# NickTravers/NeuralNetworkLibrary

Hardware: AMD Instinct MI355X
Metric: ResNet-34 224x224 training throughput (Learner.train1minibatch, fwd+loss+bwd+optimizer) (higher is better)
Workload: dtype f32; 1 GPU; DogsCats ResNet-34 classifier, 224x224, bs=64 per GPU, SGD momentum 0.9, fp32; global_batch=64, image_size=224, parallelism=dp1

## Files before the change

### include/nnl.h

```cpp
#ifndef NNL_H_
#define NNL_H_

#include <stddef.h>
#include <stdint.h>

#ifdef __cplusplus
extern "C" {
#endif

typedef enum {
  NNL_OK = 0,
  NNL_ERR_INVALID_ARG = -1,
  NNL_ERR_HIP = -2,
  NNL_ERR_UNSUPPORTED = -3,
  NNL_ERR_WORKSPACE = -4
} nnl_status_t;

int nnl_version(void);
const char* nnl_last_error(void);
int nnl_reload_env(void);

enum { NNL_PROF_CONV_FWD = 0, NNL_PROF_CONV_DGRAD = 1, NNL_PROF_CONV_WGRAD = 2, NNL_PROF_EMBDOT = 3,
       NNL_PROF_TABULAR = 4, NNL_PROF_RETINA_LOSS = 5, NNL_PROF_LSTM = 6, NNL_PROF_SOFTMAX_CE = 7,
       NNL_PROF_ELEMENTWISE = 8, NNL_PROF_GEMM = 9, NNL_PROF_OPTIM = 10, NNL_PROF_KINDS = 11 };
// ... 48 lines not shown
int nnl_conv2d_wino_preferred(const nnl_conv_geom_t* g, int dgrad);
int nnl_wino_filter_multi(const nnl_wino_desc_t* desc, const int32_t* block_desc, int64_t n_blocks, void* stream);
int nnl_conv2d_fwd_pre(const float* x, const float* w, const float* bias, float* y, const nnl_conv_geom_t* g, int relu,
                       void* workspace, size_t workspace_bytes, int32_t* tile_counters, float* bn_partials, const float* bn_pivot,
                       int32_t* bn_rows, const float* u, void* stream);
int nnl_conv2d_dgrad_pre(const float* dy, const float* wt, float* dx, const nnl_conv_geom_t* g, const float* addend,
                         void* workspace, size_t workspace_bytes, int32_t* tile_counters, const float* u, void* stream);
size_t nnl_debug_conv_wino_workspace_bytes(int N, int H, int W, int C, int K);
int nnl_debug_conv_wino_fwd(const float* x, const float* filt, const float* bias, const float* add, float* y, void* ws,
                            size_t ws_bytes, int32_t* counters, long n_counters, float* bn_part, const float* bn_pivot, int N,
                            int H, int W, int C, int K, int relu, int flip, void* stream);
size_t nnl_debug_conv_wino2_workspace_bytes(int N, int H, int W, int C, int K);
int nnl_debug_conv_wino2_fwd(const float* x, const float* filt, const float* bias, const float* add, float* y, void* ws,
                            size_t ws_bytes, int32_t* counters, long n_counters, float* bn_part, const float* bn_pivot, int N,
                            int H, int W, int C, int K, int relu, int flip, void* stream);
int nnl_debug_conv_plan_times(int N, int H, int W, int C, int K, double* out);
size_t nnl_conv2d_wgrad_workspace_bytes(const nnl_conv_geom_t* g);
int nnl_conv2d_wgrad(const float* x, const float* dy, float* dw, const nnl_conv_geom_t* g, void* workspace,
                     size_t workspace_bytes, void* stream);
size_t nnl_colsum_workspace_bytes(int64_t rows, int64_t cols);
int nnl_sum_tensors(const float* const* src, int n, float* out, int64_t numel, void* stream);
int nnl_colsum(const float* a, float* out, int64_t rows, int64_t cols, void* workspace, size_t workspace_bytes,
               void* stream);
int nnl_relu_gate_colsum(const float* dy, const float* y, float* g, float* colsum, int64_t rows, int64_t cols, void* workspace,
                         size_t workspace_bytes, void* stream);
int nnl_act_gate_colsum(const float* dy, const float* y, float* g, float* colsum, int64_t rows, int64_t cols, int act,
                        void* workspace, size_t workspace_bytes, void* stream);

size_t nnl_bn_workspace_bytes(int64_t rows, int64_t C);
int nnl_bn_fwd(const float* x, const float* gamma, const float* beta, const float* residual, float* y,
// ... 141 lines not shown
```

### neuralnetworklibrary_amd/_lib.py

```python
import ctypes as C
import os

import torch

_HERE = os.path.dirname(os.path.abspath(__file__))
LIB_PATH = os.environ.get('NNL_LIB_PATH') or os.path.join(_HERE, 'libnnl_hip.so')

if not os.path.exists(LIB_PATH):
    raise ImportError(
        f"{LIB_PATH} not found: build it with `python -c 'import __graft_entry__ as g; g.build()'` "
        "(or `make -C neuralnetworklibrary_amd/csrc`). There is no CPU fallback for the HIP hot path.")

lib = C.CDLL(LIB_PATH)

c_p = C.c_void_p
i32, i64, f32, f64 = C.c_int32, C.c_int64, C.c_float, C.c_double
sz = C.c_size_t


class ConvGeom(C.Structure):
    _fields_ = [('N', i32), ('H', i32), ('W', i32), ('C', i32), ('K', i32), ('R', i32), ('S', i32),
                ('stride', i32), ('pad', i32), ('P', i32), ('Q', i32)]


# ... 12 lines not shown
                                     c_p, c_p]),
    'nnl_embdotbias_bwd_workspace_bytes': (sz, [i64]),
    'nnl_embdotbias_bwd': (C.c_int, [c_p, c_p, c_p, c_p, c_p, c_p, c_p, c_p, c_p, i64, i64, i64, i64, C.c_int,
                                     f32, f32, c_p, sz, c_p]),
    'nnl_conv2d_fwd_workspace_bytes': (sz, [C.POINTER(ConvGeom)]),
    'nnl_conv2d_dgrad_workspace_bytes': (sz, [C.POINTER(ConvGeom)]),
    'nnl_conv2d_tile_counters': (i64, []),
    'nnl_conv2d_wino_preferred': (C.c_int, [C.POINTER(ConvGeom), C.c_int]),
    'nnl_wino_filter_multi': (C.c_int, [c_p, c_p, i64, c_p]),
    'nnl_conv2d_fwd_pre': (C.c_int, [c_p, c_p, c_p, c_p, C.POINTER(ConvGeom), C.c_int, c_p, sz, c_p, c_p, c_p, C.POINTER(i32), c_p, c_p]),
    'nnl_conv2d_dgrad_pre': (C.c_int, [c_p, c_p, c_p, C.POINTER(ConvGeom), c_p, c_p, sz, c_p, c_p, c_p]),
    'nnl_debug_conv_wino_workspace_bytes': (sz, [C.c_int] * 5),
    'nnl_debug_conv_wino_fwd': (C.c_int, [c_p] * 6 + [sz, c_p, C.c_long, c_p, c_p] + [C.c_int] * 7 + [c_p]),
    'nnl_debug_conv_wino2_workspace_bytes': (sz, [C.c_int] * 5),
    'nnl_debug_conv_wino2_fwd': (C.c_int, [c_p] * 6 + [sz, c_p, C.c_long, c_p, c_p] + [C.c_int] * 7 + [c_p]),
    'nnl_debug_conv_plan_times': (C.c_int, [C.c_int] * 5 + [C.POINTER(C.c_double)]),
    'nnl_conv2d_fwd': (C.c_int, [c_p, c_p, c_p, c_p, C.POINTER(ConvGeom), C.c_int, c_p, sz, c_p, c_p, c_p, C.POINTER(i32), c_p]),
    'nnl_conv2d_weight_transpose': (C.c_int, [c_p, c_p, C.c_int, C.c_int, C.c_int, C.c_int, c_p]),
    'nnl_conv2d_weight_transpose_multi': (C.c_int, [c_p, c_p, i64, f64, c_p]),
    'nnl_conv2d_dgrad': (C.c_int, [c_p, c_p, c_p, C.POINTER(ConvGeom), c_p, c_p, sz, c_p, c_p]),
    'nnl_conv2d_wgrad_workspace_bytes': (sz, [C.POINTER(ConvGeom)]),
    'nnl_conv2d_wgrad': (C.c_int, [c_p, c_p, c_p, C.POINTER(ConvGeom), c_p, sz, c_p]),
    'nnl_colsum_workspace_bytes': (sz, [i64, i64]),
    'nnl_colsum': (C.c_int, [c_p, c_p, i64, i64, c_p, sz, c_p]),
    'nnl_relu_gate_colsum': (C.c_int, [c_p, c_p, c_p, c_p, i64, i64, c_p, sz, c_p]),
    'nnl_conv2d_fwd_add_up2': (C.c_int, [c_p, c_p, c_p, c_p, c_p, C.POINTER(ConvGeom), c_p]),
    'nnl_upsample2_bwd': (C.c_int, [c_p, c_p, i64, i64, i64, i64, c_p]),
    'nnl_act_gate_colsum': (C.c_int, [c_p, c_p, c_p, c_p, i64, i64, C.c_int, c_p, sz, c_p]),
    'nnl_maxpool2d_fwd': (C.c_int, [c_p, c_p, c_p, i64, i64, i64, i64, i64, i64, C.c_int, C.c_int, C.c_int, c_p]),
    'nnl_maxpool2d_bwd': (C.c_int, [c_p, c_p, c_p, i64, i64, i64, i64, i64, i64, C.c_int, C.c_int, C.c_int, c_p]),
# ... 121 lines not shown
```

### neuralnetworklibrary_amd/csrc/wino2.hip

```cpp
#include "wino.h"
#include "wino_filter.h"
#include "igemm_taps.h"
#include <algorithm>

namespace {

constexpr int kCUs = 256;

template <int POL>
__device__ __forceinline__ f32x4 buf_load4_spol(__amdgpu_buffer_rsrc_t rsrc, unsigned voff, unsigned soff) {
  const i32x4 v = __builtin_bit_cast(i32x4, __builtin_amdgcn_raw_buffer_load_b128(rsrc, (int)voff, (int)soff, POL));
  return __builtin_bit_cast(f32x4, v);
}

struct Wino2Params {
  const float* a;
  const float* b;
  float* y;
  const float* bias;
  const float* add;
  unsigned a_bytes, b_bytes;
  int H, W, C, H2, W2;
  int ch;
  int prio;
// ... 5 lines not shown
  int bal, main_ks, n_main_tiles, tail_slices, tail_row0;
  float* main_out; long main_slab_stride;
  float* tail_out; long tail_slab_stride;
  int* tile_counters;
  float* bn_part; const float* bn_pivot;
  int pos_cs;
};

__global__ void wino2_filter_kernel(const float* __restrict__ w, float* __restrict__ u, long KC, int C, int flip) {
  const long i = (long)blockIdx.x * blockDim.x + threadIdx.x;
  if (i >= KC) return;
  const long c = i % C, k = i / C;
  wino2_filter_item(w + k * 9 * C + c, u + k * 16 * C + c, C, flip);
}

template <int BK, int OCC, bool POS = false>
__global__ __launch_bounds__(256, OCC) void wino2_kernel(const Wino2Params p) {
  constexpr int BM = 64, BN = 64, BKP = BK + 4, KC = BK / 4, RPP = 256 / KC, PA = BM / RPP, PB = BN / RPP;
  __shared__ __attribute__((aligned(16))) float lds[2][(BM + BN) * BKP];
  const int tid = threadIdx.x, lane = tid & 63, wave = tid >> 6, wm = wave >> 1, wn = wave & 1;
  int logical, kslice = 0, nslices = 1, row0 = 0;
  bool in_tail = false;
  if (p.bal) {
    const int nmb = p.n_main_tiles * p.main_ks;
    if ((int)blockIdx.x < nmb) {
      const int u = nnl_xcd_remap(blockIdx.x, nmb);
      logical = u / p.main_ks;
      kslice = u - logical * p.main_ks;
      nslices = p.main_ks;
    } else {
      const int tb = (int)blockIdx.x - nmb;
      const int t = tb / p.tail_slices;
      kslice = tb - t * p.tail_slices;
      logical = p.n_main_tiles + t;
      nslices = p.tail_slices;
// ... 13 lines not shown
  int a_off[PA];
  unsigned rmask[PA], cmask[PA];
#pragma unroll
  for (int i = 0; i < PA; ++i) {
    const int m = m0 + lrow + i * RPP;
    const bool valid = m < p.M4;
    const int mm = valid ? m : 0;
    const int l2 = qdiv(mm, p.mg_W2), j = mm - l2 * p.W2;
    const int n = qdiv(l2, p.mg_H2), ii = l2 - n * p.H2;
    a_off[i] = (((n * p.H + 2 * ii - 1) * p.W + 2 * j - 1) * p.C + kc * 4) * 4;
    unsigned rm = 0, cm = 0;
    if (valid) {
      for (int a = 0; a < 4; ++a) if ((unsigned)(2 * ii - 1 + a) < (unsigned)p.H) rm |= 1u << a;
      for (int a = 0; a < 4; ++a) if ((unsigned)(2 * j - 1 + a) < (unsigned)p.W) cm |= 1u << a;
    }
    rmask[i] = rm; cmask[i] = cm;
  }
  unsigned b_off[PB];
#pragma unroll
  for (int i = 0; i < PB; ++i) {
    const int nr = n0 + lrow + i * RPP;
    b_off[i] = nr < p.Nc ? (unsigned)(nr * 16 * p.C + kc * 4) * 4u : 0xFFFFFFFFu;
  }
  unsigned v00[PA], v01[PA], v10[PA], v11[PA], b_tap = 0;
  float sr = 1.f, sc = 1.f;
  auto set_pos = [&](int t) {
    const int xi = t >> 2, nu = t & 3;
    const int ra_ = xi, rb_ = xi < 2 ? 2 : 1;
    const int ca = nu, cb = nu < 2 ? 2 : 1;
    sr = xi == 1 ? 1.f : -1.f;
    sc = nu == 1 ? 1.f : -1.f;
    b_tap = (unsigned)(t * p.C) * 4u;
    const int wc = p.W * p.C * 4, c4 = p.C * 4;
#pragma unroll
    for (int i = 0; i < PA; ++i) {
      const bool ra_ok = (rmask[i] >> ra_) & 1u, rb_ok = (rmask[i] >> rb_) & 1u;
      const bool ca_ok = (cmask[i] >> ca) & 1u, cb_ok = (cmask[i] >> cb) & 1u;
      v00[i] = (ra_ok && ca_ok) ? (unsigned)(a_off[i] + ra_ * wc + ca * c4) : 0xFFFFFFFFu;
      v01[i] = (ra_ok && cb_ok) ? (unsigned)(a_off[i] + ra_ * wc + cb * c4) : 0xFFFFFFFFu;
      v10[i] = (rb_ok && ca_ok) ? (unsigned)(a_off[i] + rb_ * wc + ca * c4) : 0xFFFFFFFFu;
      v11[i] = (rb_ok && cb_ok) ? (unsigned)(a_off[i] + rb_ * wc + cb * c4) : 0xFFFFFFFFu;
    }
  };
  f32x4 r00[PA], r01[PA], r10[PA], r11[PA], rb[PB];
  auto load_tile = [&](int c0) {
#pragma unroll
    for (int i = 0; i < PA; ++i) {
      r00[i] = buf_load4(ra_src, v00[i], (unsigned)c0 * 4u); r01[i] = buf_load4(ra_src, v01[i], (unsigned)c0 * 4u);
      r10[i] = buf_load4(ra_src, v10[i], (unsigned)c0 * 4u); r11[i] = buf_load4(ra_src, v11[i], (unsigned)c0 * 4u);
    }
#pragma unroll
    for (int i = 0; i < PB; ++i) rb[i] = buf_load4(rb_src, b_off[i], b_tap + (unsigned)c0 * 4u);
  };
  float sr_ld = 1.f, sc_ld = 1.f;
  auto store_tile = [&](int buf) {
    float* As = lds[buf];
    float* Bs = As + BM * BKP;
#pragma unroll
    for (int i = 0; i < PA; ++i) {
      f32x4 v;
#pragma unroll
      for (int e = 0; e < 4; ++e)
        v[e] = __builtin_fmaf(sr_ld, __builtin_fmaf(sc_ld, r11[i][e], r10[i][e]), __builtin_fmaf(sc_ld, r01[i][e], r00[i][e]));
      *reinterpret_cast<f32x4*>(As + (lrow + i * RPP) * BKP + kc * 4) = v;
    }
#pragma unroll
    for (int i = 0; i < PB; ++i) *reinterpret_cast<f32x4*>(Bs + (lrow + i * RPP) * BKP + kc * 4) = rb[i];
// ... 99 lines not shown
#pragma unroll
        for (int e = 0; e < 16; ++e) y10[e] = __builtin_fmaf(k10, tm[e], y10[e]);
      }
      if (k11 != 0.f) {
#pragma unroll
        for (int e = 0; e < 16; ++e) y11[e] = __builtin_fmaf(k11, tm[e], y11[e]);
      }
#pragma unroll
      for (int e = 0; e < 16; ++e) tm[e] = 0.f;
      cs_cur = 0; t_cur = (t_cur + 1) & 15;
    }
  }

  const int col_l = lane & 31, row_h = (lane >> 5) * 4;
  constexpr int kSc1 = 1 << 4;
  if constexpr (POS) {
    __shared__ int ticket;
    const long sstride = p.main_slab_stride;
    const __amdgpu_buffer_rsrc_t rs = __builtin_amdgcn_make_buffer_rsrc(p.main_out, 0, (int)((long)nslices * sstride * 4), 0x00020000);
    const int cl = n0 + wn * 32 + col_l;
#pragma unroll
    for (int e = 0; e < 16; ++e) {
      const int row = m0 + wm * 32 + (e & 3) + 8 * (e >> 2) + row_h;
      const long off = (long)kslice * sstride + (long)row * p.Nc + cl;
      const bool ok = row < p.M4 && cl < p.Nc;
      __builtin_amdgcn_raw_buffer_store_b32(__float_as_uint(tm[e]), rs, ok ? (int)(off * 4) : -1, 0, kSc1);
    }
    asm volatile("s_waitcnt vmcnt(0)" ::: "memory");
    __syncthreads();
    if (tid == 0) ticket = __hip_atomic_fetch_add(&p.tile_counters[logical], 1, __ATOMIC_RELAXED, __HIP_MEMORY_SCOPE_AGENT);
    __syncthreads();
    if (ticket != nslices - 1) return;
    if (tid == 0) __hip_atomic_store(&p.tile_counters[logical], 0, __ATOMIC_RELAXED, __HIP_MEMORY_SCOPE_AGENT);
    float fs1[4] = {0.f, 0.f, 0.f, 0.f}, fs2[4] = {0.f, 0.f, 0.f, 0.f};
    const int c4 = n0 + (tid & 15) * 4, cs = p.pos_cs;
    const int wrow = p.W * p.Nc;
    auto item_off = [&](int k4, bool& ok) {
      const int row = m0 + (tid >> 4) + 16 * k4;
      ok = row < p.M4 && c4 < p.Nc;
      return ok ? (unsigned)(((long)row * p.Nc + c4) * 4) : 0xFFFFFFFFu;
    };
    auto finish_item = [&](int k4, f32x4 (&m)[16]) {
      const int row = m0 + (tid >> 4) + 16 * k4;
      f32x4 r0[4], r1[4];
#pragma unroll
      for (int xi = 0; xi < 4; ++xi) {
        r0[xi] = (m[xi * 4 + 0] + m[xi * 4 + 1]) + m[xi * 4 + 2];
        r1[xi] = (m[xi * 4 + 1] - m[xi * 4 + 2]) + m[xi * 4 + 3];
      }
      f32x4 out[4];
      out[0] = (r0[0] + r0[1]) + r0[2];
      out[1] = (r1[0] + r1[1]) + r1[2];
      out[2] = (r0[1] - r0[2]) + r0[3];
      out[3] = (r1[1] - r1[2]) + r1[3];
      const int l2 = qdiv(row, p.mg_W2), j = row - l2 * p.W2;
      const int n = qdiv(l2, p.mg_H2), ii = l2 - n * p.H2;
      const long ob = (((long)n * p.H + 2 * ii) * p.W + 2 * j) * p.Nc + c4;
      const bool h1 = 2 * ii + 1 < p.H, w1 = 2 * j + 1 < p.W;
// ... 21 lines not shown
      f32x4 ma[16];
#pragma unroll
      for (int t = 0; t < 16; ++t) ma[t] = buf_load4_spol<kSc1>(rs, oa, (unsigned)((long)(t * cs) * sstride * 4));
      for (int sl = 1; sl < cs; ++sl) {
#pragma unroll
        for (int t0 = 0; t0 < 16; t0 += 8) {
          f32x4 pa[8];
#pragma unroll
          for (int t = 0; t < 8; ++t) pa[t] = buf_load4_spol<kSc1>(rs, oa, (unsigned)((long)((t0 + t) * cs + sl) * sstride * 4));
#pragma unroll
          for (int t = 0; t < 8; ++t) ma[t0 + t] += pa[t];
        }
      }
      finish_item(k4, ma);
    }
    if (p.bn_part) {
      __syncthreads();
      float* red = &lds[0][0];
#pragma unroll
      for (int e = 0; e < 4; ++e) {
        red[(((tid >> 4) * 64) + (tid & 15) * 4 + e) * 2 + 0] = fs1[e];
        red[(((tid >> 4) * 64) + (tid & 15) * 4 + e) * 2 + 1] = fs2[e];
      }
      __syncthreads();
      if (tid < 64 && n0 + tid < p.Nc) {
        float a = 0.f, b = 0.f;
        for (int r = 0; r < 16; ++r) { a += red[(r * 64 + tid) * 2]; b += red[(r * 64 + tid) * 2 + 1]; }
        p.bn_part[((long)tile_m * p.Nc + n0 + tid) * 2 + 0] = a;
        p.bn_part[((long)tile_m * p.Nc + n0 + tid) * 2 + 1] = b;
      }
    }
    return;
  }
  if (partial) {
    __shared__ int ticket;
    float* const base = in_tail ? p.tail_out : p.main_out;
    const long sstride = in_tail ? p.tail_slab_stride : p.main_slab_stride;
    const __amdgpu_buffer_rsrc_t rs = __builtin_amdgcn_make_buffer_rsrc(base, 0, (int)((long)nslices * sstride * 4), 0x00020000);
    const int cl = n0 + wn * 32 + col_l;
#pragma unroll
    for (int e = 0; e < 16; ++e) {
      const int row = m0 + wm * 32 + (e & 3) + 8 * (e >> 2) + row_h;
      const long off = (long)kslice * sstride + (long)(row - row0) * 4 * p.Nc + cl;
      const bool ok = row < p.M4 && cl < p.Nc;
      __builtin_amdgcn_raw_buffer_store_b32(__float_as_uint(y00[e]), rs, ok ? (int)(off * 4) : -1, 0, kSc1);
      __builtin_amdgcn_raw_buffer_store_b32(__float_as_uint(y01[e]), rs, ok ? (int)((off + p.Nc) * 4) : -1, 0, kSc1);
      __builtin_amdgcn_raw_buffer_store_b32(__float_as_uint(y10[e]), rs, ok ? (int)((off + 2 * p.Nc) * 4) : -1, 0, kSc1);
      __builtin_amdgcn_raw_buffer_store_b32(__float_as_uint(y11[e]), rs, ok ? (int)((off + 3 * p.Nc) * 4) : -1, 0, kSc1);
    }
    asm volatile("s_waitcnt vmcnt(0)" ::: "memory");
    __syncthreads();
    if (tid == 0) ticket = __hip_atomic_fetch_add(&p.tile_counters[logical], 1, __ATOMIC_RELAXED, __HIP_MEMORY_SCOPE_AGENT);
    __syncthreads();
    if (ticket != nslices - 1) return;
    if (tid == 0) __hip_atomic_store(&p.tile_counters[logical], 0, __ATOMIC_RELAXED, __HIP_MEMORY_SCOPE_AGENT);
    float fs1[4] = {0.f, 0.f, 0.f, 0.f}, fs2[4] = {0.f, 0.f, 0.f, 0.f};
    const int h = (tid >> 4) & 3, c4 = n0 + (tid & 15) * 4;
    for (int k16 = 0; k16 < 16; ++k16) {
      const int row = m0 + (tid >> 6) + 4 * k16;
      if (row >= p.M4 || c4 >= p.Nc) continue;
      const int l2 = qdiv(row, p.mg_W2), j = row - l2 * p.W2;
      const int n = qdiv(l2, p.mg_H2), ii = l2 - n * p.H2;
      const int oh = 2 * ii + (h >> 1), ow = 2 * j + (h & 1);
      if (oh >= p.H || ow >= p.W) continue;
      f32x4 v = {0.f, 0.f, 0.f, 0.f};
      for (int sl0 = 0; sl0 < nslices; sl0 += 8) {
        f32x4 part[8];
#pragma unroll
        for (int sl = 0; sl < 8; ++sl)
          if (sl0 + sl < nslices) part[sl] = buf_load4_pol(rs, (unsigned)(((long)(sl0 + sl) * sstride + ((long)(row - row0) * 4 + h) * p.Nc + c4) * 4), kSc1);
#pragma unroll
        for (int sl = 0; sl < 8; ++sl)
          if (sl0 + sl < nslices) v += part[sl];
      }
      const long o = (((long)n * p.H + oh) * p.W + ow) * p.Nc + c4;
      if (p.bias) v += *reinterpret_cast<const f32x4*>(p.bias + c4);
      if (p.add) v += *reinterpret_cast<const f32x4*>(p.add + o);
      if (p.relu == 1) { v[0] = fmaxf(v[0], 0.f); v[1] = fmaxf(v[1], 0.f); v[2] = fmaxf(v[2], 0.f); v[3] = fmaxf(v[3], 0.f); }
      *reinterpret_cast<f32x4*>(p.y + o) = v;
      if (p.bn_part) {
        const f32x4 pv = *reinterpret_cast<const f32x4*>(p.bn_pivot + c4);
#pragma unroll
        for (int e = 0; e < 4; ++e) { const float d = v[e] - pv[e]; fs1[e] += d; fs2[e] += d * d; }
      }
    }
    if (p.bn_part) {
      __syncthreads();
      float* red = &lds[0][0];
#pragma unroll
      for (int e = 0; e < 4; ++e) {
        red[(((tid >> 4) * 64) + (tid & 15) * 4 + e) * 2 + 0] = fs1[e];
        red[(((tid >> 4) * 64) + (tid & 15) * 4 + e) * 2 + 1] = fs2[e];
      }
      __syncthreads();
      if (tid < 64 && n0 + tid < p.Nc) {
        float a = 0.f, b = 0.f;
        for (int r = 0; r < 16; ++r) { a += red[(r * 64 + tid) * 2]; b += red[(r * 64 + tid) * 2 + 1]; }
        p.bn_part[((long)tile_m * p.Nc + n0 + tid) * 2 + 0] = a;
        p.bn_part[((long)tile_m * p.Nc + n0 + tid) * 2 + 1] = b;
      }
    }
    return;
  }
  constexpr int LDT = 68;
  float* tl = &lds[0][0];
  float fs1[4] = {0.f, 0.f, 0.f, 0.f}, fs2[4] = {0.f, 0.f, 0.f, 0.f};
  const int c4 = n0 + (tid & 15) * 4;
  int pb[4];
  unsigned okm[4];
#pragma unroll
  for (int k4 = 0; k4 < 4; ++k4) {
    const int row = m0 + (tid >> 4) + 16 * k4;
    const int l2 = qdiv(row, p.mg_W2), j = row - l2 * p.W2;
    const int n = qdiv(l2, p.mg_H2), ii = l2 - n * p.H2;
    pb[k4] = ((n * p.H + 2 * ii) * p.W + 2 * j) * p.Nc + c4;
    const bool ok = row < p.M4 && c4 < p.Nc, h1 = 2 * ii + 1 < p.H, w1 = 2 * j + 1 < p.W;
    okm[k4] = ok ? (1u | (w1 ? 2u : 0u) | (h1 ? 4u : 0u) | ((h1 && w1) ? 8u : 0u)) : 0u;
  }
  const int wrow = p.W * p.Nc;
#pragma unroll
  for (int h = 0; h < 4; ++h) {
    if (h) __syncthreads();
#pragma unroll
    for (int e = 0; e < 16; ++e)
      tl[(wm * 32 + (e & 3) + 8 * (e >> 2) + row_h) * LDT + wn * 32 + col_l] = h == 0 ? y00[e] : (h == 1 ? y01[e] : (h == 2 ? y10[e] : y11[e]));
    __syncthreads();
#pragma unroll
    for (int k4 = 0; k4 < 4; ++k4) {
      if (!((okm[k4] >> h) & 1u)) continue;
      f32x4 v = *reinterpret_cast<const f32x4*>(tl + ((tid >> 4) + 16 * k4) * LDT + (tid & 15) * 4);
      const int o = pb[k4] + (h >> 1) * wrow + (h & 1) * p.Nc;
      if (p.bias) v += *reinterpret_cast<const f32x4*>(p.bias + c4);
      if (p.add) v += *reinterpret_cast<const f32x4*>(p.add + o);
      if (p.relu == 1) { v[0] = fmaxf(v[0], 0.f); v[1] = fmaxf(v[1], 0.f); v[2] = fmaxf(v[2], 0.f); v[3] = fmaxf(v[3], 0.f); }
      *reinterpret_cast<f32x4*>(p.y + o) = v;
      if (p.bn_part) {
        const f32x4 pv = *reinterpret_cast<const f32x4*>(p.bn_pivot + c4);
#pragma unroll
        for (int e = 0; e < 4; ++e) { const float d = v[e] - pv[e]; fs1[e] += d; fs2[e] += d * d; }
      }
    }
  }
  if (p.bn_part) {
    __syncthreads();
    float* red = &lds[0][0];
#pragma unroll
    for (int e = 0; e < 4; ++e) {
      red[(((tid >> 4) * 64) + (tid & 15) * 4 + e) * 2 + 0] = fs1[e];
      red[(((tid >> 4) * 64) + (tid & 15) * 4 + e) * 2 + 1] = fs2[e];
    }
    __syncthreads();
    if (tid < 64 && n0 + tid < p.Nc) {
      float a = 0.f, b = 0.f;
      for (int r = 0; r < 16; ++r) { a += red[(r * 64 + tid) * 2]; b += red[(r * 64 + tid) * 2 + 1]; }
      p.bn_part[((long)tile_m * p.Nc + n0 + tid) * 2 + 0] = a;
      p.bn_part[((long)tile_m * p.Nc + n0 + tid) * 2 + 1] = b;
    }
  }
}

struct W2Plan {
  int bk, on, main_ks, n_main_tiles, tail_slices, tail_row0;
  size_t main_floats, tail_floats;
  double t_us;
  int pos_cs;
};

double w2_pos_cost(long T, long M4, int Nc, int C, int cs) {
  const double a = 0.363, b = 0.490, tfix = 4.0;
  const long occ = 4, nwg = T * 16 * cs, I = (C / 32) / cs;
  const long nb = nnl_cdiv(nwg, (long)kCUs);
  const double c = (double)(nb < occ ? nb : occ);
  const double slab_b = 2.0 * 16 * cs * (double)M4 * Nc * 4;
  return nb * I * (b + a / c) + tfix * nb / c + slab_b / 11.7e6 + (3.0 + 1.5 * cs) + 4.0;
}

double w2_cost(long T, long gn, long M4, int Nc, long I, int bk, int ks, int S, W2Plan* out) {
  const double a = bk == 32 ? 0.363 : 0.226, b = bk == 32 ? 0.490 : 0.243, tfix = bk == 32 ? 12.3 : 15.0;
  const long occ = bk == 16 ? 4 : 3;
  long n_main = ((T * ks / kCUs) * kCUs / ks / gn) * gn;
  if (n_main > T) n_main = T;
  const long tail = T - n_main;
  if (tail == 0 && S > 1) return -1.0;
  const long m = nnl_cdiv(n_main * ks, (long)kCUs), q = nnl_cdiv(tail * S, (long)kCUs);
  const long W = m * nnl_cdiv(I, (long)ks) + q * nnl_cdiv(I, (long)S), nb = m + q;
  const double c = (double)(nb < occ ? nb : occ);
  const long row0 = (n_main / gn) * 64 < M4 ? (n_main / gn) * 64 : M4;
  const double main_b = ks > 1 ? (2.0 * ks + 1) * row0 * 4 * Nc * 4 : 0;
  const double tail_b = (S > 1 && tail) ? (2.0 * S + 1) * (M4 - row0) * 4 * Nc * 4 : 0;
  if (out) {
    out->bk = bk; out->on = (ks > 1 || (S > 1 && tail)) ? 1 : 0;
    out->main_ks = ks; out->n_main_tiles = (int)n_main; out->tail_slices = tail ? S : 1; out->tail_row0 = (int)row0;
    out->main_floats = ks > 1 ? (size_t)ks * row0 * 4 * Nc : 0;
    out->tail_floats = (S > 1 && tail) ? (size_t)S * (M4 - row0) * 4 * Nc : 0;
  }
  return W * (b + a / c) + tfix * nb / c + (main_b + tail_b) / 11.7e6 + 10.0;
}

W2Plan wino2_plan(long M4, int Nc, int C) {
  W2Plan best{};
  const long gm = nnl_cdiv(M4, 64), gn = nnl_cdiv(Nc, 64), T = gm * gn;
  const int f_ks = NNL_ENV_INT("NNL_WINO_PLAN_KS", 0), f_S = NNL_ENV_INT("NNL_WINO_PLAN_S", 0);
  const bool balance = NNL_ENV_INT("NNL_WINO_BALANCE", 1) != 0;
  double best_t = 1e300;
  static const int kSlices[] = {1, 2, 3, 4, 6, 8, 12, 16};
  for (int bk = 16; bk <= 32; bk *= 2) {
    if (C % bk != 0) continue;
    const long I = 16L * (C / bk);
    for (int ks = 1; ks <= 4; ks *= 2) {
      if (ks > 1 && (!balance || I / ks < 8)) break;
      if (f_ks > 0 && ks != f_ks && balance) continue;
      for (int S : kSlices) {
        if (S > 1 && (!balance || I / S < 4)) break;
        W2Plan cand{};
        const double t = w2_cost(T, gn, M4, Nc, I, bk, ks, S, &cand);
        if (t < 0) break;
        if (f_S > 0 && balance && cand.n_main_tiles < T && S != f_S) continue;
        if (t < best_t) { best_t = t; best = cand; best.t_us = t; }
      }
    }
  }
  if (best_t == 1e300) {
    best.t_us = w2_cost(T, gn, M4, Nc, 16L * (C / 16), 16, 1, 1, &best);
    best_t = best.t_us;
  }
  const int e_pos = NNL_ENV_INT("NNL_WINO2_POS", -1);
  if (e_pos != 0 && (balance || e_pos > 0) && C % 32 == 0) {
    const int csteps = C / 32;
    double pt = 1e300; int pcs = 0;
    for (int cs = 1; cs <= 8; cs *= 2) {
      if (csteps % cs != 0 || (csteps / cs < 2 && cs > 1)) break;
      if (e_pos > 0 && cs != e_pos && csteps % e_pos == 0) continue;
      const size_t fl = (size_t)16 * cs * M4 * Nc;
      if (fl * sizeof(float) >= (1UL << 31)) break;
      const double t = w2_pos_cost(T, M4, Nc, C, cs);
      if (t < pt) { pt = t; pcs = cs; }
    }
    if (pcs && (e_pos > 0 || pt < best_t)) {
      best = W2Plan{};
      best.bk = 32; best.on = 1; best.main_ks = 16 * pcs; best.n_main_tiles = (int)T; best.tail_slices = 1; best.tail_row0 = (int)M4;
      best.main_floats = (size_t)16 * pcs * M4 * Nc; best.tail_floats = 0; best.t_us = pt; best.pos_cs = pcs;
    }
  }
  return best;
}

size_t align4(size_t floats) { return (floats + 3) & ~(size_t)3; }

long quads(int N, int H, int W) { return (long)N * ((H + 1) / 2) * ((W + 1) / 2); }

}

bool nnl_wino2_ok(int N, int H, int W, int Cin, int Nc, int R, int S, int stride, int pad) {
  if (R != 3 || S != 3 || stride != 1 || pad != 1 || W < 2 || H < 2 || Cin % 16 != 0 || Nc % 4 != 0) return false;
  const long a_b = (long)N * H * W * Cin * 4, b_b = (long)Nc * 16 * Cin * 4, y_b = (long)N * H * W * Nc * 4;
  if ((quads(N, H, W) + 128) * (long)std::max((W + 1) / 2, (H + 1) / 2) >= (1L << 32)) return false;
  return a_b < (1L << 31) && b_b < (1L << 31) && y_b < (1L << 31);
}

double nnl_wino2_plan_time_us(int N, int H, int W, int Cin, int Nc) { return wino2_plan(quads(N, H, W), Nc, Cin).t_us; }
bool nnl_wino2_plan_is_pos(int N, int H, int W, int Cin, int Nc) { return wino2_plan(quads(N, H, W), Nc, Cin).pos_cs > 0; }

size_t nnl_wino2_workspace_bytes(int N, int H, int W, int Cin, int Nc) {
  const W2Plan pl = wino2_plan(quads(N, H, W), Nc, Cin);
  return (align4((size_t)Nc * 16 * Cin) + (pl.on ? pl.main_floats + pl.tail_floats : 0)) * sizeof(float);
}

int nnl_wino2_bn_rows(int N, int H, int W) { return (int)nnl_cdiv(quads(N, H, W), 64L); }

int nnl_wino2_launch(const WinoProblem& q, void* ws, size_t ws_bytes, int* tile_counters, long n_counters, hipStream_t s) {
  const long M4 = quads(q.N, q.H, q.W);
  const size_t u_floats = align4((size_t)q.Nc * 16 * q.Cin);
  if (ws == nullptr || ws_bytes < u_floats * sizeof(float)) return nnl_set_error(NNL_ERR_WORKSPACE, "wino2: workspace too small");
  float* u = (float*)ws;
  if (q.u_pre == nullptr) {
    const long KC = (long)q.Nc * q.Cin;
// ... 1 lines not shown
    NNL_CHECK_LAUNCH();
  }
  Wino2Params p{};
  p.a = q.in; p.b = q.u_pre ? q.u_pre : u; p.y = q.out; p.bias = q.bias; p.add = q.add;
  p.a_bytes = (unsigned)((long)q.N * q.H * q.W * q.Cin * 4); p.b_bytes = (unsigned)((long)q.Nc * 16 * q.Cin * 4);
  {
    const int e_ch = NNL_ENV_INT("NNL_WINO2_CHUNK", 0);
    p.ch = (e_ch > 0 && e_ch % 32 == 0 && q.Cin % e_ch == 0) ? e_ch : q.Cin;
    p.prio = 0;
  }
  p.H = q.H; p.W = q.W; p.C = q.Cin; p.H2 = (q.H + 1) / 2; p.W2 = (q.W + 1) / 2; p.M4 = (int)M4; p.Nc = q.Nc; p.relu = q.relu;
  {
    auto magic = [](int d) { return d <= 1 ? 0u : (unsigned)(((1ULL << 32) + d - 1) / (unsigned)d); };
    p.mg_W2 = magic(p.W2); p.mg_H2 = magic(p.H2);
  }
  p.grid_m = (int)nnl_cdiv(M4, 64L); p.grid_n = (int)nnl_cdiv(q.Nc, 64);
  p.bn_part = q.bn_part; p.bn_pivot = q.bn_pivot;
  const long T = (long)p.grid_m * p.grid_n;
  W2Plan pl = wino2_plan(M4, q.Nc, q.Cin);
  if (pl.on && (tile_counters == nullptr || T > n_counters || ws_bytes < (u_floats + pl.main_floats + pl.tail_floats) * sizeof(float) ||
                pl.main_floats * sizeof(float) >= (1UL << 31) || pl.tail_floats * sizeof(float) >= (1UL << 31))) {
    if (pl.pos_cs) {
      const int bk = q.Cin % 32 == 0 ? 32 : 16;
      w2_cost(T, p.grid_n, M4, q.Nc, 16L * (q.Cin / bk), bk, 1, 1, &pl);
      pl.pos_cs = 0;
    }
    pl.on = 0;
  }
  unsigned grid = (unsigned)T;
  if (pl.pos_cs) {
    p.bal = 1; p.main_ks = pl.main_ks; p.n_main_tiles = pl.n_main_tiles; p.tail_slices = 1; p.tail_row0 = (int)M4;
    p.main_out = u + u_floats; p.main_slab_stride = M4 * q.Nc; p.tile_counters = tile_counters; p.pos_cs = pl.pos_cs;
    grid = (unsigned)(T * pl.main_ks);
    hipLaunchKernelGGL((wino2_kernel<32, 4, true>), dim3(grid), dim3(256), 0, s, p);
    NNL_CHECK_LAUNCH();
    return NNL_OK;
  }
  if (pl.on) {
    p.bal = 1; p.main_ks = pl.main_ks; p.n_main_tiles = pl.n_main_tiles; p.tail_slices = pl.tail_slices; p.tail_row0 = pl.tail_row0;
    p.main_out = u + u_floats; p.main_slab_stride = (long)pl.tail_row0 * 4 * q.Nc;
    p.tail_out = p.main_out + pl.main_floats; p.tail_slab_stride = (long)(M4 - pl.tail_row0) * 4 * q.Nc;
    p.tile_counters = tile_counters;
    grid = (unsigned)(pl.n_main_tiles * pl.main_ks + (T - pl.n_main_tiles) * pl.tail_slices);
  }
  if (pl.bk == 32) hipLaunchKernelGGL((wino2_kernel<32, 3>), dim3(grid), dim3(256), 0, s, p);
  else hipLaunchKernelGGL((wino2_kernel<16, 4>), dim3(grid), dim3(256), 0, s, p);
  NNL_CHECK_LAUNCH();
  return NNL_OK;
}

extern "C" size_t nnl_debug_conv_wino2_workspace_bytes(int N, int H, int W, int C, int K) { return nnl_wino2_workspace_bytes(N, H, W, C, K); }
extern "C" int nnl_debug_conv_wino2_fwd(const float* x, const float* w, const float* bias, const float* add, float* y, void* ws,
                                        size_t ws_bytes, int32_t* counters, long n_counters, float* bn_part, const float* bn_pivot, int N,
                                        int H, int W, int C, int K, int relu, int flip, void* stream) {
  NNL_CHECK_ARG(nnl_wino2_ok(N, H, W, C, K, 3, 3, 1, 1), "wino2: unsupported shape");
  WinoProblem q{};
  q.in = x; q.filt = w; q.out = y; q.bias = bias; q.add = add; q.N = N; q.H = H; q.W = W; q.Cin = C; q.Nc = K; q.relu = relu; q.flip = flip;
  q.bn_part = bn_part; q.bn_pivot = bn_pivot;
  return nnl_wino2_launch(q, ws, ws_bytes, counters, n_counters, (hipStream_t)stream);
}
```

Before: 5543 images/s.

## Add 128-wide N tile variant to Winograd F(2,3) conv kernel with planner choice

Adds a BN=128 (512-thread) instantiation of the wino2 GEMM kernel, both in the regular and the position-split paths, so each A tile is reused across twice as many output channels. The cost-model planner now weighs wide against narrow tiles with its own constants and a margin, and is enabled by default when Nc is a multiple of 128. The BN reduction epilogue is pulled out into a shared lambda, and a debug entry point reports the chosen plan. In exchange, the wide tile needs more LDS and registers, which means lower occupancy, and its cost constants are guesses that may pick it where it is slower.

```diff
diff --git a/include/nnl.h b/include/nnl.h
--- a/include/nnl.h
+++ b/include/nnl.h
@@ -86,6 +86,7 @@
 int nnl_debug_conv_wino2_fwd(const float* x, const float* filt, const float* bias, const float* add, float* y, void* ws,
                             size_t ws_bytes, int32_t* counters, long n_counters, float* bn_part, const float* bn_pivot, int N,
                             int H, int W, int C, int K, int relu, int flip, void* stream);
+int nnl_debug_conv_wino2_plan(int N, int H, int W, int C, int K, int32_t* out);
 int nnl_debug_conv_plan_times(int N, int H, int W, int C, int K, double* out);
 size_t nnl_conv2d_wgrad_workspace_bytes(const nnl_conv_geom_t* g);
 int nnl_conv2d_wgrad(const float* x, const float* dy, float* dw, const nnl_conv_geom_t* g, void* workspace,
diff --git a/neuralnetworklibrary_amd/_lib.py b/neuralnetworklibrary_amd/_lib.py
--- a/neuralnetworklibrary_amd/_lib.py
+++ b/neuralnetworklibrary_amd/_lib.py
@@ -50,6 +50,7 @@
     'nnl_debug_conv_wino_fwd': (C.c_int, [c_p] * 6 + [sz, c_p, C.c_long, c_p, c_p] + [C.c_int] * 7 + [c_p]),
     'nnl_debug_conv_wino2_workspace_bytes': (sz, [C.c_int] * 5),
     'nnl_debug_conv_wino2_fwd': (C.c_int, [c_p] * 6 + [sz, c_p, C.c_long, c_p, c_p] + [C.c_int] * 7 + [c_p]),
+    'nnl_debug_conv_wino2_plan': (C.c_int, [C.c_int] * 5 + [C.POINTER(i32)]),
     'nnl_debug_conv_plan_times': (C.c_int, [C.c_int] * 5 + [C.POINTER(C.c_double)]),
     'nnl_conv2d_fwd': (C.c_int, [c_p, c_p, c_p, c_p, C.POINTER(ConvGeom), C.c_int, c_p, sz, c_p, c_p, c_p, C.POINTER(i32), c_p]),
     'nnl_conv2d_weight_transpose': (C.c_int, [c_p, c_p, C.c_int, C.c_int, C.c_int, C.c_int, c_p]),
diff --git a/neuralnetworklibrary_amd/csrc/wino2.hip b/neuralnetworklibrary_amd/csrc/wino2.hip
--- a/neuralnetworklibrary_amd/csrc/wino2.hip
+++ b/neuralnetworklibrary_amd/csrc/wino2.hip
@@ -43,11 +43,14 @@
   wino2_filter_item(w + k * 9 * C + c, u + k * 16 * C + c, C, flip);
 }
 
-template <int BK, int OCC, bool POS = false>
-__global__ __launch_bounds__(256, OCC) void wino2_kernel(const Wino2Params p) {
-  constexpr int BM = 64, BN = 64, BKP = BK + 4, KC = BK / 4, RPP = 256 / KC, PA = BM / RPP, PB = BN / RPP;
+template <int BK, int OCC, bool POS = false, int BN = 64>
+__global__ __launch_bounds__(BN * 4, OCC) void wino2_kernel(const Wino2Params p) {
+  constexpr int NT = BN * 4, WN = BN / 32, TPR = BN / 4;
+  constexpr int BM = 64, BKP = BK + 4, KC = BK / 4, RPP = NT / KC, PA = BM / RPP, PB = BN / RPP;
+  static_assert(BN == 64 || (BN == 128 && BK == 32), "the wide tile is BK 32 only");
+  static_assert(PA >= 1 && PB >= 1 && NT / TPR == 16, "staging / epilogue thread maps");
   __shared__ __attribute__((aligned(16))) float lds[2][(BM + BN) * BKP];
-  const int tid = threadIdx.x, lane = tid & 63, wave = tid >> 6, wm = wave >> 1, wn = wave & 1;
+  const int tid = threadIdx.x, lane = tid & 63, wave = BN == 128 ? __builtin_amdgcn_readfirstlane(tid >> 6) : tid >> 6, wm = wave / WN, wn = wave % WN;
   int logical, kslice = 0, nslices = 1, row0 = 0;
   bool in_tail = false;
   if (p.bal) {
@@ -91,7 +94,7 @@
       for (int a = 0; a < 4; ++a) if ((unsigned)(2 * ii - 1 + a) < (unsigned)p.H) rm |= 1u << a;
       for (int a = 0; a < 4; ++a) if ((unsigned)(2 * j - 1 + a) < (unsigned)p.W) cm |= 1u << a;
     }
-    rmask[i] = rm; cmask[i] = cm;
+    rmask[i] = BN == 128 ? (rm | cm << 4) : rm; cmask[i] = cm;
   }
   unsigned b_off[PB];
 #pragma unroll
@@ -111,8 +114,9 @@
     const int wc = p.W * p.C * 4, c4 = p.C * 4;
 #pragma unroll
     for (int i = 0; i < PA; ++i) {
+      const unsigned cm = BN == 128 ? rmask[i] >> 4 : cmask[i];
       const bool ra_ok = (rmask[i] >> ra_) & 1u, rb_ok = (rmask[i] >> rb_) & 1u;
-      const bool ca_ok = (cmask[i] >> ca) & 1u, cb_ok = (cmask[i] >> cb) & 1u;
+      const bool ca_ok = (cm >> ca) & 1u, cb_ok = (cm >> cb) & 1u;
       v00[i] = (ra_ok && ca_ok) ? (unsigned)(a_off[i] + ra_ * wc + ca * c4) : 0xFFFFFFFFu;
       v01[i] = (ra_ok && cb_ok) ? (unsigned)(a_off[i] + ra_ * wc + cb * c4) : 0xFFFFFFFFu;
       v10[i] = (rb_ok && ca_ok) ? (unsigned)(a_off[i] + rb_ * wc + ca * c4) : 0xFFFFFFFFu;
@@ -127,7 +131,12 @@
       r10[i] = buf_load4(ra_src, v10[i], (unsigned)c0 * 4u); r11[i] = buf_load4(ra_src, v11[i], (unsigned)c0 * 4u);
     }
 #pragma unroll
-    for (int i = 0; i < PB; ++i) rb[i] = buf_load4(rb_src, b_off[i], b_tap + (unsigned)c0 * 4u);
+    for (int i = 0; i < PB; ++i) {
+      if constexpr (BN == 128)
+        rb[i] = buf_load4(rb_src, b_off[0], b_tap + (unsigned)c0 * 4u + (unsigned)(i * RPP * 16 * p.C) * 4u);
+      else
+        rb[i] = buf_load4(rb_src, b_off[i], b_tap + (unsigned)c0 * 4u);
+    }
   };
   float sr_ld = 1.f, sc_ld = 1.f;
   auto store_tile = [&](int buf) {
@@ -257,6 +266,22 @@
 
   const int col_l = lane & 31, row_h = (lane >> 5) * 4;
   constexpr int kSc1 = 1 << 4;
+  auto bn_reduce = [&](const float (&fs1)[4], const float (&fs2)[4]) {
+    __syncthreads();
+    float* red = &lds[0][0];
+#pragma unroll
+    for (int e = 0; e < 4; ++e) {
+      red[(((tid / TPR) * BN) + (tid % TPR) * 4 + e) * 2 + 0] = fs1[e];
+      red[(((tid / TPR) * BN) + (tid % TPR) * 4 + e) * 2 + 1] = fs2[e];
+    }
+    __syncthreads();
+    if (tid < BN && n0 + tid < p.Nc) {
+      float a = 0.f, b = 0.f;
+      for (int r = 0; r < 16; ++r) { a += red[(r * BN + tid) * 2]; b += red[(r * BN + tid) * 2 + 1]; }
+      p.bn_part[((long)tile_m * p.Nc + n0 + tid) * 2 + 0] = a;
+      p.bn_part[((long)tile_m * p.Nc + n0 + tid) * 2 + 1] = b;
+    }
+  };
   if constexpr (POS) {
     __shared__ int ticket;
     const long sstride = p.main_slab_stride;
@@ -276,15 +301,15 @@
     if (ticket != nslices - 1) return;
     if (tid == 0) __hip_atomic_store(&p.tile_counters[logical], 0, __ATOMIC_RELAXED, __HIP_MEMORY_SCOPE_AGENT);
     float fs1[4] = {0.f, 0.f, 0.f, 0.f}, fs2[4] = {0.f, 0.f, 0.f, 0.f};
-    const int c4 = n0 + (tid & 15) * 4, cs = p.pos_cs;
+    const int c4 = n0 + (tid % TPR) * 4, cs = p.pos_cs;
     const int wrow = p.W * p.Nc;
     auto item_off = [&](int k4, bool& ok) {
-      const int row = m0 + (tid >> 4) + 16 * k4;
+      const int row = m0 + tid / TPR + 16 * k4;
       ok = row < p.M4 && c4 < p.Nc;
       return ok ? (unsigned)(((long)row * p.Nc + c4) * 4) : 0xFFFFFFFFu;
     };
     auto finish_item = [&](int k4, f32x4 (&m)[16]) {
-      const int row = m0 + (tid >> 4) + 16 * k4;
+      const int row = m0 + tid / TPR + 16 * k4;
       f32x4 r0[4], r1[4];
 #pragma unroll
       for (int xi = 0; xi < 4; ++xi) {
@@ -336,22 +361,7 @@
       }
       finish_item(k4, ma);
     }
-    if (p.bn_part) {
-      __syncthreads();
-      float* red = &lds[0][0];
-#pragma unroll
-      for (int e = 0; e < 4; ++e) {
-        red[(((tid >> 4) * 64) + (tid & 15) * 4 + e) * 2 + 0] = fs1[e];
-        red[(((tid >> 4) * 64) + (tid & 15) * 4 + e) * 2 + 1] = fs2[e];
-      }
-      __syncthreads();
-      if (tid < 64 && n0 + tid < p.Nc) {
-        float a = 0.f, b = 0.f;
-        for (int r = 0; r < 16; ++r) { a += red[(r * 64 + tid) * 2]; b += red[(r * 64 + tid) * 2 + 1]; }
-        p.bn_part[((long)tile_m * p.Nc + n0 + tid) * 2 + 0] = a;
-        p.bn_part[((long)tile_m * p.Nc + n0 + tid) * 2 + 1] = b;
-      }
-    }
+    if (p.bn_part) bn_reduce(fs1, fs2);
     return;
   }
   if (partial) {
@@ -377,9 +387,9 @@
     if (ticket != nslices - 1) return;
     if (tid == 0) __hip_atomic_store(&p.tile_counters[logical], 0, __ATOMIC_RELAXED, __HIP_MEMORY_SCOPE_AGENT);
     float fs1[4] = {0.f, 0.f, 0.f, 0.f}, fs2[4] = {0.f, 0.f, 0.f, 0.f};
-    const int h = (tid >> 4) & 3, c4 = n0 + (tid & 15) * 4;
+    const int h = (tid / TPR) & 3, c4 = n0 + (tid % TPR) * 4;
     for (int k16 = 0; k16 < 16; ++k16) {
-      const int row = m0 + (tid >> 6) + 4 * k16;
+      const int row = m0 + tid / (4 * TPR) + 4 * k16;
       if (row >= p.M4 || c4 >= p.Nc) continue;
       const int l2 = qdiv(row, p.mg_W2), j = row - l2 * p.W2;
       const int n = qdiv(l2, p.mg_H2), ii = l2 - n * p.H2;
@@ -406,33 +416,19 @@
         for (int e = 0; e < 4; ++e) { const float d = v[e] - pv[e]; fs1[e] += d; fs2[e] += d * d; }
       }
     }
-    if (p.bn_part) {
-      __syncthreads();
-      float* red = &lds[0][0];
-#pragma unroll
-      for (int e = 0; e < 4; ++e) {
-        red[(((tid >> 4) * 64) + (tid & 15) * 4 + e) * 2 + 0] = fs1[e];
-        red[(((tid >> 4) * 64) + (tid & 15) * 4 + e) * 2 + 1] = fs2[e];
-      }
-      __syncthreads();
-      if (tid < 64 && n0 + tid < p.Nc) {
-        float a = 0.f, b = 0.f;
-        for (int r = 0; r < 16; ++r) { a += red[(r * 64 + tid) * 2]; b += red[(r * 64 + tid) * 2 + 1]; }
-        p.bn_part[((long)tile_m * p.Nc + n0 + tid) * 2 + 0] = a;
-        p.bn_part[((long)tile_m * p.Nc + n0 + tid) * 2 + 1] = b;
-      }
-    }
+    if (p.bn_part) bn_reduce(fs1, fs2);
     return;
   }
-  constexpr int LDT = 68;
+  constexpr int LDT = BN + 4;
+  static_assert(64 * LDT <= 2 * (BM + BN) * BKP, "epilogue tile exceeds the LDS");
   float* tl = &lds[0][0];
   float fs1[4] = {0.f, 0.f, 0.f, 0.f}, fs2[4] = {0.f, 0.f, 0.f, 0.f};
-  const int c4 = n0 + (tid & 15) * 4;
+  const int c4 = n0 + (tid % TPR) * 4;
   int pb[4];
   unsigned okm[4];
 #pragma unroll
   for (int k4 = 0; k4 < 4; ++k4) {
-    const int row = m0 + (tid >> 4) + 16 * k4;
+    const int row = m0 + tid / TPR + 16 * k4;
     const int l2 = qdiv(row, p.mg_W2), j = row - l2 * p.W2;
     const int n = qdiv(l2, p.mg_H2), ii = l2 - n * p.H2;
     pb[k4] = ((n * p.H + 2 * ii) * p.W + 2 * j) * p.Nc + c4;
@@ -450,7 +446,7 @@
 #pragma unroll
     for (int k4 = 0; k4 < 4; ++k4) {
       if (!((okm[k4] >> h) & 1u)) continue;
-      f32x4 v = *reinterpret_cast<const f32x4*>(tl + ((tid >> 4) + 16 * k4) * LDT + (tid & 15) * 4);
+      f32x4 v = *reinterpret_cast<const f32x4*>(tl + (tid / TPR + 16 * k4) * LDT + (tid % TPR) * 4);
       const int o = pb[k4] + (h >> 1) * wrow + (h & 1) * p.Nc;
       if (p.bias) v += *reinterpret_cast<const f32x4*>(p.bias + c4);
       if (p.add) v += *reinterpret_cast<const f32x4*>(p.add + o);
@@ -463,22 +459,7 @@
       }
     }
   }
-  if (p.bn_part) {
-    __syncthreads();
-    float* red = &lds[0][0];
-#pragma unroll
-    for (int e = 0; e < 4; ++e) {
-      red[(((tid >> 4) * 64) + (tid & 15) * 4 + e) * 2 + 0] = fs1[e];
-      red[(((tid >> 4) * 64) + (tid & 15) * 4 + e) * 2 + 1] = fs2[e];
-    }
-    __syncthreads();
-    if (tid < 64 && n0 + tid < p.Nc) {
-      float a = 0.f, b = 0.f;
-      for (int r = 0; r < 16; ++r) { a += red[(r * 64 + tid) * 2]; b += red[(r * 64 + tid) * 2 + 1]; }
-      p.bn_part[((long)tile_m * p.Nc + n0 + tid) * 2 + 0] = a;
-      p.bn_part[((long)tile_m * p.Nc + n0 + tid) * 2 + 1] = b;
-    }
-  }
+  if (p.bn_part) bn_reduce(fs1, fs2);
 }
 
 struct W2Plan {
@@ -486,20 +467,24 @@
   size_t main_floats, tail_floats;
   double t_us;
   int pos_cs;
+  int wide;
 };
 
-double w2_pos_cost(long T, long M4, int Nc, int C, int cs) {
-  const double a = 0.363, b = 0.490, tfix = 4.0;
-  const long occ = 4, nwg = T * 16 * cs, I = (C / 32) / cs;
+constexpr double kWideA = 0.363, kWideB = 0.95, kWideTfix = 14.0, kWideMargin = 0.98;
+
+double w2_pos_cost(long T, long M4, int Nc, int C, int cs, bool wide = false) {
+  const double a = wide ? kWideA : 0.363, b = wide ? kWideB : 0.490, tfix = 4.0;
+  const long occ = wide ? 2 : 4, nwg = T * 16 * cs, I = (C / 32) / cs;
   const long nb = nnl_cdiv(nwg, (long)kCUs);
   const double c = (double)(nb < occ ? nb : occ);
   const double slab_b = 2.0 * 16 * cs * (double)M4 * Nc * 4;
   return nb * I * (b + a / c) + tfix * nb / c + slab_b / 11.7e6 + (3.0 + 1.5 * cs) + 4.0;
 }
 
-double w2_cost(long T, long gn, long M4, int Nc, long I, int bk, int ks, int S, W2Plan* out) {
-  const double a = bk == 32 ? 0.363 : 0.226, b = bk == 32 ? 0.490 : 0.243, tfix = bk == 32 ? 12.3 : 15.0;
-  const long occ = bk == 16 ? 4 : 3;
+double w2_cost(long T, long gn, long M4, int Nc, long I, int bk, int ks, int S, W2Plan* out, bool wide = false) {
+  const double a = wide ? kWideA : (bk == 32 ? 0.363 : 0.226), b = wide ? kWideB : (bk == 32 ? 0.490 : 0.243);
+  const double tfix = wide ? kWideTfix : (bk == 32 ? 12.3 : 15.0);
+  const long occ = wide ? 1 : (bk == 16 ? 4 : 3);
   long n_main = ((T * ks / kCUs) * kCUs / ks / gn) * gn;
   if (n_main > T) n_main = T;
   const long tail = T - n_main;
@@ -515,53 +500,69 @@
     out->main_ks = ks; out->n_main_tiles = (int)n_main; out->tail_slices = tail ? S : 1; out->tail_row0 = (int)row0;
     out->main_floats = ks > 1 ? (size_t)ks * row0 * 4 * Nc : 0;
     out->tail_floats = (S > 1 && tail) ? (size_t)S * (M4 - row0) * 4 * Nc : 0;
+    out->wide = wide ? 1 : 0;
   }
   return W * (b + a / c) + tfix * nb / c + (main_b + tail_b) / 11.7e6 + 10.0;
 }
 
-W2Plan wino2_plan(long M4, int Nc, int C) {
+W2Plan wino2_plan(long M4, int Nc, int C, bool allow_wide = true) {
   W2Plan best{};
-  const long gm = nnl_cdiv(M4, 64), gn = nnl_cdiv(Nc, 64), T = gm * gn;
+  const int e_wide = allow_wide ? NNL_ENV_INT("NNL_WINO2_WIDE", -1) : 0;
+  const bool wide_ok = e_wide != 0 && Nc % 128 == 0 && C % 32 == 0;
+  const long gm = nnl_cdiv(M4, 64);
   const int f_ks = NNL_ENV_INT("NNL_WINO_PLAN_KS", 0), f_S = NNL_ENV_INT("NNL_WINO_PLAN_S", 0);
   const bool balance = NNL_ENV_INT("NNL_WINO_BALANCE", 1) != 0;
   double best_t = 1e300;
   static const int kSlices[] = {1, 2, 3, 4, 6, 8, 12, 16};
-  for (int bk = 16; bk <= 32; bk *= 2) {
-    if (C % bk != 0) continue;
-    const long I = 16L * (C / bk);
-    for (int ks = 1; ks <= 4; ks *= 2) {
-      if (ks > 1 && (!balance || I / ks < 8)) break;
-      if (f_ks > 0 && ks != f_ks && balance) continue;
-      for (int S : kSlices) {
-        if (S > 1 && (!balance || I / S < 4)) break;
-        W2Plan cand{};
-        const double t = w2_cost(T, gn, M4, Nc, I, bk, ks, S, &cand);
-        if (t < 0) break;
-        if (f_S > 0 && balance && cand.n_main_tiles < T && S != f_S) continue;
-        if (t < best_t) { best_t = t; best = cand; best.t_us = t; }
+  auto beats = [&](double t, int wide, double bt, int bt_wide) { return t < ((wide && !bt_wide && e_wide < 0) ? kWideMargin : 1.0) * bt; };
+  for (int wide = 0; wide <= (wide_ok ? 1 : 0); ++wide) {
+    if (!wide && wide_ok && e_wide > 0) continue;
+    const long gn = nnl_cdiv(Nc, wide ? 128 : 64), T = gm * gn;
+    for (int bk = wide ? 32 : 16; bk <= 32; bk *= 2) {
+      if (C % bk != 0) continue;
+      const long I = 16L * (C / bk);
+      for (int ks = 1; ks <= 4; ks *= 2) {
+        if (ks > 1 && (!balance || I / ks < 8)) break;
+        if (f_ks > 0 && ks != f_ks && balance) continue;
+        for (int S : kSlices) {
+          if (S > 1 && (!balance || I / S < 4)) break;
+          W2Plan cand{};
+          const double t = w2_cost(T, gn, M4, Nc, I, bk, ks, S, &cand, wide);
+          if (t < 0) break;
+          if (f_S > 0 && balance && cand.n_main_tiles < T && S != f_S) continue;
+          if (beats(t, wide, best_t, best.wide)) { best_t = t; best = cand; best.t_us = t; }
+        }
       }
     }
   }
   if (best_t == 1e300) {
-    best.t_us = w2_cost(T, gn, M4, Nc, 16L * (C / 16), 16, 1, 1, &best);
+    const bool w = wide_ok && e_wide > 0;
+    const long gn = nnl_cdiv(Nc, w ? 128 : 64);
+    const int bk = w ? 32 : 16;
+    best.t_us = w2_cost(gm * gn, gn, M4, Nc, 16L * (C / bk), bk, 1, 1, &best, w);
     best_t = best.t_us;
   }
   const int e_pos = NNL_ENV_INT("NNL_WINO2_POS", -1);
   if (e_pos != 0 && (balance || e_pos > 0) && C % 32 == 0) {
     const int csteps = C / 32;
-    double pt = 1e300; int pcs = 0;
-    for (int cs = 1; cs <= 8; cs *= 2) {
-      if (csteps % cs != 0 || (csteps / cs < 2 && cs > 1)) break;
-      if (e_pos > 0 && cs != e_pos && csteps % e_pos == 0) continue;
-      const size_t fl = (size_t)16 * cs * M4 * Nc;
-      if (fl * sizeof(float) >= (1UL << 31)) break;
-      const double t = w2_pos_cost(T, M4, Nc, C, cs);
-      if (t < pt) { pt = t; pcs = cs; }
-    }
-    if (pcs && (e_pos > 0 || pt < best_t)) {
+    double pt = 1e300; int pcs = 0, pwide = 0;
+    for (int wide = 0; wide <= (wide_ok ? 1 : 0); ++wide) {
+      if (!wide && wide_ok && e_wide > 0) continue;
+      const long T = gm * nnl_cdiv(Nc, wide ? 128 : 64);
+      for (int cs = 1; cs <= 8; cs *= 2) {
+        if (csteps % cs != 0 || (csteps / cs < 2 && cs > 1)) break;
+        if (e_pos > 0 && cs != e_pos && csteps % e_pos == 0) continue;
+        const size_t fl = (size_t)16 * cs * M4 * Nc;
+        if (fl * sizeof(float) >= (1UL << 31)) break;
+        const double t = w2_pos_cost(T, M4, Nc, C, cs, wide);
+        if (!pcs || beats(t, wide, pt, pwide)) { pt = t; pcs = cs; pwide = wide; }
+      }
+    }
+    if (pcs && (e_pos > 0 || beats(pt, pwide, best_t, best.wide))) {
       best = W2Plan{};
-      best.bk = 32; best.on = 1; best.main_ks = 16 * pcs; best.n_main_tiles = (int)T; best.tail_slices = 1; best.tail_row0 = (int)M4;
-      best.main_floats = (size_t)16 * pcs * M4 * Nc; best.tail_floats = 0; best.t_us = pt; best.pos_cs = pcs;
+      best.bk = 32; best.on = 1; best.main_ks = 16 * pcs; best.n_main_tiles = (int)(gm * nnl_cdiv(Nc, pwide ? 128 : 64));
+      best.tail_slices = 1; best.tail_row0 = (int)M4;
+      best.main_floats = (size_t)16 * pcs * M4 * Nc; best.tail_floats = 0; best.t_us = pt; best.pos_cs = pcs; best.wide = pwide;
     }
   }
   return best;
@@ -580,8 +581,8 @@
   return a_b < (1L << 31) && b_b < (1L << 31) && y_b < (1L << 31);
 }
 
-double nnl_wino2_plan_time_us(int N, int H, int W, int Cin, int Nc) { return wino2_plan(quads(N, H, W), Nc, Cin).t_us; }
-bool nnl_wino2_plan_is_pos(int N, int H, int W, int Cin, int Nc) { return wino2_plan(quads(N, H, W), Nc, Cin).pos_cs > 0; }
+double nnl_wino2_plan_time_us(int N, int H, int W, int Cin, int Nc) { return wino2_plan(quads(N, H, W), Nc, Cin, false).t_us; }
+bool nnl_wino2_plan_is_pos(int N, int H, int W, int Cin, int Nc) { return wino2_plan(quads(N, H, W), Nc, Cin, false).pos_cs > 0; }
 
 size_t nnl_wino2_workspace_bytes(int N, int H, int W, int Cin, int Nc) {
   const W2Plan pl = wino2_plan(quads(N, H, W), Nc, Cin);
@@ -613,15 +614,15 @@
     auto magic = [](int d) { return d <= 1 ? 0u : (unsigned)(((1ULL << 32) + d - 1) / (unsigned)d); };
     p.mg_W2 = magic(p.W2); p.mg_H2 = magic(p.H2);
   }
-  p.grid_m = (int)nnl_cdiv(M4, 64L); p.grid_n = (int)nnl_cdiv(q.Nc, 64);
+  W2Plan pl = wino2_plan(M4, q.Nc, q.Cin);
+  p.grid_m = (int)nnl_cdiv(M4, 64L); p.grid_n = (int)nnl_cdiv(q.Nc, pl.wide ? 128 : 64);
   p.bn_part = q.bn_part; p.bn_pivot = q.bn_pivot;
   const long T = (long)p.grid_m * p.grid_n;
-  W2Plan pl = wino2_plan(M4, q.Nc, q.Cin);
   if (pl.on && (tile_counters == nullptr || T > n_counters || ws_bytes < (u_floats + pl.main_floats + pl.tail_floats) * sizeof(float) ||
                 pl.main_floats * sizeof(float) >= (1UL << 31) || pl.tail_floats * sizeof(float) >= (1UL << 31))) {
     if (pl.pos_cs) {
       const int bk = q.Cin % 32 == 0 ? 32 : 16;
-      w2_cost(T, p.grid_n, M4, q.Nc, 16L * (q.Cin / bk), bk, 1, 1, &pl);
+      w2_cost(T, p.grid_n, M4, q.Nc, 16L * (q.Cin / bk), bk, 1, 1, &pl, pl.wide && bk == 32);
       pl.pos_cs = 0;
     }
     pl.on = 0;
@@ -631,7 +632,8 @@
     p.bal = 1; p.main_ks = pl.main_ks; p.n_main_tiles = pl.n_main_tiles; p.tail_slices = 1; p.tail_row0 = (int)M4;
     p.main_out = u + u_floats; p.main_slab_stride = M4 * q.Nc; p.tile_counters = tile_counters; p.pos_cs = pl.pos_cs;
     grid = (unsigned)(T * pl.main_ks);
-    hipLaunchKernelGGL((wino2_kernel<32, 4, true>), dim3(grid), dim3(256), 0, s, p);
+    if (pl.wide) hipLaunchKernelGGL((wino2_kernel<32, 4, true, 128>), dim3(grid), dim3(512), 0, s, p);
+    else hipLaunchKernelGGL((wino2_kernel<32, 4, true>), dim3(grid), dim3(256), 0, s, p);
     NNL_CHECK_LAUNCH();
     return NNL_OK;
   }
@@ -642,7 +644,8 @@
     p.tile_counters = tile_counters;
     grid = (unsigned)(pl.n_main_tiles * pl.main_ks + (T - pl.n_main_tiles) * pl.tail_slices);
   }
-  if (pl.bk == 32) hipLaunchKernelGGL((wino2_kernel<32, 3>), dim3(grid), dim3(256), 0, s, p);
+  if (pl.wide) hipLaunchKernelGGL((wino2_kernel<32, 2, false, 128>), dim3(grid), dim3(512), 0, s, p);
+  else if (pl.bk == 32) hipLaunchKernelGGL((wino2_kernel<32, 3>), dim3(grid), dim3(256), 0, s, p);
   else hipLaunchKernelGGL((wino2_kernel<16, 4>), dim3(grid), dim3(256), 0, s, p);
   NNL_CHECK_LAUNCH();
   return NNL_OK;
@@ -658,3 +661,11 @@
   q.bn_part = bn_part; q.bn_pivot = bn_pivot;
   return nnl_wino2_launch(q, ws, ws_bytes, counters, n_counters, (hipStream_t)stream);
 }
+
+extern "C" int nnl_debug_conv_wino2_plan(int N, int H, int W, int C, int K, int32_t* out) {
+  NNL_CHECK_ARG(out && nnl_wino2_ok(N, H, W, C, K, 3, 3, 1, 1), "wino2: unsupported shape");
+  const W2Plan pl = wino2_plan(quads(N, H, W), K, C);
+  out[0] = pl.bk; out[1] = pl.wide ? 128 : 64; out[2] = pl.pos_cs;
+  out[3] = pl.on ? pl.main_ks : 1; out[4] = pl.n_main_tiles; out[5] = pl.on ? pl.tail_slices : 1;
+  return NNL_OK;
+}
```

Result: no change. 5539 images/s (median of 2 runs) (-0.1%).
